# iPERDance/iPERCore

Hardware: AMD Instinct MI355X
Metric: synthesized frames/sec at 512x512 (run_imitator) (higher is better)
Workload: dtype f32; 1 GPU; run_imitator 512x512 single src/ref pair, 300-frame reference clip frame-sharded over 1 GPU(s), AttLWB-SPADE generator fp32 (BASELINE configs[1] at N = 1, configs[2] at N = 8); poses=imitate, image_size=512, frame_batch=300, frame_batch_requested=384, world_size=1, parallelism=frame-shard x1, batches_in_flight=1, weights=random-init (seeded) of the real architecture, 36,276,992 params

## Files before the change

include/lwg_hip.h:

```cpp
#ifndef LWG_HIP_H
#define LWG_HIP_H

#include <stddef.h>
#include <stdint.h>

#ifdef __cplusplus
extern "C" {
#endif

typedef void* lwg_stream_t;

#define LWG_ABI_VERSION 10
int lwg_abi_version(void);

#define LWG_MAX_TAPS 52
enum { LWG_EPI_NONE = 0, LWG_EPI_RESIDUAL = 1, LWG_EPI_SPADE = 2 };
enum { LWG_ACTIVATION_NONE = 0, LWG_ACTIVATION_RELU = 1, LWG_ACTIVATION_TANH = 2, LWG_ACTIVATION_SIGMOID = 3 };
#define LWG_ACTIVATION_RELU_MASK 5
enum { LWG_DT_F32 = 0, LWG_DT_BF16 = 1,
       LWG_DT_F32_Q4 = 2 };

typedef struct LwgConvArgs {
    const float* x0;
    const float* x1;
    int C0, C1;
    int B, H, W;
    int OH, OW;
    int M;
    int stride;
    int ntaps;
    int cshift;
    const float* w;
    int N;
    const float* bias;
    float* y;
    int YH, YW, YC, ycoff;
    int omul, ooy, oox;
    int epi;
    int act;
    const float* res;
    const float* xn;
    const float* mean;
    const float* rstd;
    int xdt;
    int ydt;
    signed char dy[LWG_MAX_TAPS];
    signed char dx[LWG_MAX_TAPS];
} LwgConvArgs;

int lwg_conv2d_nhwc_f32(const LwgConvArgs* args, lwg_stream_t stream);
size_t lwg_conv2d_ws_floats(const LwgConvArgs* args);
int lwg_conv2d_nhwc_f32_ws(const LwgConvArgs* args, float* ws, lwg_stream_t stream);
int lwg_conv_slice_count(const LwgConvArgs* args);

int lwg_conv2d_nhwc_bf16(const LwgConvArgs* args, lwg_stream_t stream);
int lwg_conv2d_winograd_f32(const LwgConvArgs* args, lwg_stream_t stream);
size_t lwg_conv2d_winograd_ws_floats(const LwgConvArgs* args);
int lwg_conv2d_winograd_f32_ws(const LwgConvArgs* args, float* ws, lwg_stream_t stream);
int lwg_conv2d_winograd_plan(const LwgConvArgs* args, int with_ws, long long* blocks, int* slices, int* nbv, int* workgroups);
int lwg_winograd_panel_f32(const float* wpanel, float* upk, int Cin, int N, const int* tap9, lwg_stream_t stream);
typedef struct LwgWinoDesc {
    const float* wpanel;
    float* upk;
    int Cin, N, first_block;
    int tap9[9];
} LwgWinoDesc;
int lwg_winograd_panels_f32(const LwgWinoDesc* descs_dev, int ndesc, int total_blocks, lwg_stream_t stream);
int lwg_conv2d_winograd4_f32(const LwgConvArgs* args, lwg_stream_t stream);
int lwg_winograd4_panel_f32(const float* wpanel, float* upk, int Cin, int N, const int* tap9, lwg_stream_t stream);
int lwg_conv2d_nhwc_bf16_hr(const LwgConvArgs* args, lwg_stream_t stream);
int lwg_conv2d_nhwc_c8_bf16(const LwgConvArgs* args, lwg_stream_t stream);
int lwg_conv_transpose4_nhwc_bf16(const LwgConvArgs* args, lwg_stream_t stream);
int lwg_conv_transpose4_nhwc_f32(const LwgConvArgs* args, lwg_stream_t stream);
int lwg_conv_transpose4_is_one_grid(const LwgConvArgs* args);
int lwg_conv_transpose4_winograd_f32(const LwgConvArgs* args, lwg_stream_t stream);

int lwg_conv2d_nhwc_f32_split(const LwgConvArgs* args, lwg_stream_t stream);

size_t lwg_conv2d_wgrad_ws_floats(int Ktot, int N, int M);
int lwg_conv2d_wgrad_nhwc_f32(const LwgConvArgs* args, const float* dy, float* dw, float* ws, lwg_stream_t stream);
int lwg_conv2d_wgrad_unpacked_f32(const LwgConvArgs* args, const float* dy, float* ws, float* dw, int D0, int D1, int KH, int KW,
                                  int transposed, const int* kidx, int cin, int nout, float* db, lwg_stream_t stream);
int lwg_colsum_nhwc_f32(const float* x, size_t rows, int C, float* out, float* ws, lwg_stream_t stream);

int lwg_act_bwd_f32(const float* dy, const float* y, size_t n, int act, float* out, lwg_stream_t stream);
int lwg_norm_fwd_nhwc_f32(const float* x, const float* mean, const float* rstd, const float* gamma, const float* beta, int gstride,
                          int B, int HW, int C, int act, float* y, lwg_stream_t stream);
int lwg_norm_bwd_nhwc_f32(const float* dy, const float* y, const float* x, const float* mean, const float* rstd,
                          const float* gamma, int gstride, int B, int HW, int C, int act, int nsplit, float* dx, float* dgamma,
                          float* dbeta, float* ws, lwg_stream_t stream);
int lwg_adam_step_f32(float* p, const float* g, float* m, float* v, size_t n, float lr, float beta1, float beta2, float eps, int t,
                      lwg_stream_t stream);
int lwg_adam_step_dev_f32(float* p, const float* g, float* m, float* v, size_t n, float lr, float beta1, float beta2, float eps,
                          int* t_dev, lwg_stream_t stream);
int lwg_pack_panel_f32(const float* w, int D0, int D1, int KH, int KW, int transposed, const int* kidx, int ntaps, int cin,
                       int cin_pad, int nout, int n_pad, float* out, lwg_stream_t stream);
int lwg_unpack_wgrad_f32(const float* dwk, int D0, int D1, int KH, int KW, int transposed, const int* kidx, int ntaps, int cin,
                         int cin_pad, int nout, int n_pad, float* dw, lwg_stream_t stream);
typedef struct LwgPackDesc {
    const float* w;
    float* out;
    int D1, KHW, transposed, ntaps, cin, cin_pad, nout, n_pad, Kp, first_block;
    int kidx[LWG_MAX_TAPS];
} LwgPackDesc;
int lwg_pack_panels_f32(const LwgPackDesc* descs_dev, int ndesc, int total_blocks, lwg_stream_t stream);
int lwg_maxpool2_fwd_nhwc_f32(const float* x, float* y, int B, int H, int W, int C, lwg_stream_t stream);
int lwg_maxpool2_bwd_nhwc_f32(const float* x, const float* dy, float* dx, int B, int H, int W, int C, lwg_stream_t stream);
int lwg_crop_resize_bilinear_f32(const float* x, const long long* box, float* y, float* valid, int N, int C, int H, int W, int OH, int OW,
                                 lwg_stream_t stream);
int lwg_crop_resize_bilinear_bwd_f32(const float* dy, const long long* box, float* dx, int N, int C, int H, int W, int OH, int OW, lwg_stream_t stream);
int lwg_prelu_f32(const float* x, const float* slope, const float* res, size_t rows, int C, float* y, lwg_stream_t stream);
int lwg_prelu_bwd_f32(const float* x, const float* slope, const float* dy, size_t rows, int C, float* dx, lwg_stream_t stream);

int lwg_instnorm_stats_nhwc_f32(const float* x, int B, int HW, int C, float eps, float* mean, float* rstd,
                                float* ws, int nsplit, lwg_stream_t stream);
int lwg_instnorm_stats_nhwc_bf16(const void* x, int B, int HW, int C, float eps, float* mean, float* rstd, float* ws, int nsplit,
                                 lwg_stream_t stream);
int lwg_instnorm_apply_nhwc_f32(const float* x, const float* mean, const float* rstd, const float* res,
                                float* y, int B, int HW, int C, int act, lwg_stream_t stream);

int lwg_flow_resize_f32(const float* T, int n, int S, int h, int w, float* out, lwg_stream_t stream);
int lwg_lwb_attention_f32(const float* q, const float* Ks, const float* Vs, const float* bk, const float* bv,
                          const float* T, float* out, int B, int ns, int h, int w, int C, int S,
                          int src_batched, lwg_stream_t stream);
int lwg_lwb_attention_bf16(const void* q, const void* Ks, const void* Vs, const float* bk, const float* bv, const float* T, void* out,
                           int B, int ns, int h, int w, int C, int S, int src_batched, lwg_stream_t stream);
int lwg_lwb_attention_x_records(int h, int w, int C, int element_size);
int lwg_lwb_attention_x_f32(const float* x, const float* Kq, const float* kappa, const float* Vs, const float* bv, const float* T,
// ... 71 lines not shown
```

ipercore_amd/_lib.py:

```python
import ctypes
import os
import re

_HERE = os.path.dirname(os.path.abspath(__file__))
LIB_PATH = os.path.join(_HERE, "liblwg_hip.so")
HEADER_PATH = os.path.join(os.path.dirname(_HERE), "include", "lwg_hip.h")

LWG_MAX_TAPS = 52
EPI_NONE, EPI_RESIDUAL, EPI_SPADE = 0, 1, 2
ACT_NONE, ACT_RELU, ACT_TANH, ACT_SIGMOID, ACT_LRELU = 0, 1, 2, 3, 4
ACT_RELU_MASK = 5
DT_F32, DT_BF16, DT_F32_Q4 = 0, 1, 2

c_f = ctypes.c_void_p
c_i = ctypes.c_int


class LwgConvArgs(ctypes.Structure):
    _fields_ = [
        ("x0", c_f), ("x1", c_f),
        ("C0", c_i), ("C1", c_i),
        ("B", c_i), ("H", c_i), ("W", c_i),
        ("OH", c_i), ("OW", c_i),
        ("M", c_i), ("stride", c_i), ("ntaps", c_i), ("cshift", c_i),
        ("w", c_f), ("N", c_i), ("bias", c_f),
        ("y", c_f), ("YH", c_i), ("YW", c_i), ("YC", c_i), ("ycoff", c_i),
        ("omul", c_i), ("ooy", c_i), ("oox", c_i),
        ("epi", c_i), ("act", c_i),
        ("res", c_f), ("xn", c_f), ("mean", c_f), ("rstd", c_f),
        ("xdt", c_i), ("ydt", c_i),
        ("dy", ctypes.c_byte * LWG_MAX_TAPS), ("dx", ctypes.c_byte * LWG_MAX_TAPS),
    ]


class LwgWinoDesc(ctypes.Structure):
    _fields_ = [("wpanel", ctypes.c_void_p), ("upk", ctypes.c_void_p), ("Cin", c_i), ("N", c_i), ("first_block", c_i), ("tap9", c_i * 9)]


class LwgPackDesc(ctypes.Structure):
    _fields_ = [("w", c_f), ("out", c_f)] + [(n, c_i) for n in ("D1", "KHW", "transposed", "ntaps", "cin", "cin_pad", "nout", "n_pad", "Kp",
                                                               "first_block")] + [("kidx", c_i * LWG_MAX_TAPS)]


_SIGS = {
    "lwg_abi_version": (c_i, []),
    "lwg_device_cu_count": (c_i, []),
    "lwg_conv2d_nhwc_f32": (c_i, [ctypes.POINTER(LwgConvArgs), c_f]),
    "lwg_conv2d_ws_floats": (ctypes.c_size_t, [ctypes.POINTER(LwgConvArgs)]),
    "lwg_conv2d_nhwc_f32_ws": (c_i, [ctypes.POINTER(LwgConvArgs), c_f, c_f]),
    "lwg_conv2d_nhwc_bf16": (c_i, [ctypes.POINTER(LwgConvArgs), c_f]),
    "lwg_conv2d_winograd_f32": (c_i, [ctypes.POINTER(LwgConvArgs), c_f]),
    "lwg_conv2d_winograd_ws_floats": (ctypes.c_size_t, [ctypes.POINTER(LwgConvArgs)]),
    "lwg_conv2d_winograd_f32_ws": (c_i, [ctypes.POINTER(LwgConvArgs), c_f, c_f]),
    "lwg_conv2d_winograd_plan": (c_i, [ctypes.POINTER(LwgConvArgs), c_i, ctypes.POINTER(ctypes.c_longlong), ctypes.POINTER(c_i), ctypes.POINTER(c_i),
                                       ctypes.POINTER(c_i)]),
    "lwg_winograd_panel_f32": (c_i, [c_f, c_f, c_i, c_i, ctypes.POINTER(c_i), c_f]),
    "lwg_winograd_panels_f32": (c_i, [c_f, c_i, c_i, c_f]),
    "lwg_conv2d_winograd4_f32": (c_i, [ctypes.POINTER(LwgConvArgs), c_f]),
    "lwg_winograd4_panel_f32": (c_i, [c_f, c_f, c_i, c_i, ctypes.POINTER(c_i), c_f]),
    "lwg_conv2d_nhwc_bf16_hr": (c_i, [ctypes.POINTER(LwgConvArgs), c_f]),
    "lwg_conv2d_nhwc_c8_bf16": (c_i, [ctypes.POINTER(LwgConvArgs), c_f]),
    "lwg_conv_transpose4_nhwc_bf16": (c_i, [ctypes.POINTER(LwgConvArgs), c_f]),
    "lwg_conv_transpose4_nhwc_f32": (c_i, [ctypes.POINTER(LwgConvArgs), c_f]),
    "lwg_conv_transpose4_winograd_f32": (c_i, [ctypes.POINTER(LwgConvArgs), c_f]),
    "lwg_conv_transpose4_is_one_grid": (c_i, [ctypes.POINTER(LwgConvArgs)]),
    "lwg_conv_slice_count": (c_i, [ctypes.POINTER(LwgConvArgs)]),
    "lwg_conv2d_nhwc_f32_split": (c_i, [ctypes.POINTER(LwgConvArgs), c_f]),
    "lwg_conv2d_wgrad_ws_floats": (ctypes.c_size_t, [c_i, c_i, c_i]),
    "lwg_conv2d_wgrad_nhwc_f32": (c_i, [ctypes.POINTER(LwgConvArgs), c_f, c_f, c_f, c_f]),
    "lwg_conv2d_wgrad_unpacked_f32": (c_i, [ctypes.POINTER(LwgConvArgs), c_f, c_f, c_f] + [c_i] * 5 + [ctypes.POINTER(ctypes.c_int), c_i, c_i, c_f, c_f]),
    "lwg_colsum_nhwc_f32": (c_i, [c_f, ctypes.c_size_t, c_i, c_f, c_f, c_f]),
    "lwg_act_bwd_f32": (c_i, [c_f, c_f, ctypes.c_size_t, c_i, c_f, c_f]),
    "lwg_norm_fwd_nhwc_f32": (c_i, [c_f, c_f, c_f, c_f, c_f, c_i, c_i, c_i, c_i, c_i, c_f, c_f]),
    "lwg_norm_bwd_nhwc_f32": (c_i, [c_f, c_f, c_f, c_f, c_f, c_f, c_i, c_i, c_i, c_i, c_i, c_i, c_f, c_f, c_f, c_f, c_f]),
    "lwg_adam_step_f32": (c_i, [c_f, c_f, c_f, c_f, ctypes.c_size_t, ctypes.c_float, ctypes.c_float, ctypes.c_float, ctypes.c_float, c_i, c_f]),
    "lwg_adam_step_dev_f32": (c_i, [c_f, c_f, c_f, c_f, ctypes.c_size_t, ctypes.c_float, ctypes.c_float, ctypes.c_float, ctypes.c_float, c_f, c_f]),
    "lwg_pack_panel_f32": (c_i, [c_f] + [c_i] * 5 + [ctypes.POINTER(ctypes.c_int)] + [c_i] * 5 + [c_f, c_f]),
    "lwg_pack_panels_f32": (c_i, [c_f, c_i, c_i, c_f]),
    "lwg_unpack_wgrad_f32": (c_i, [c_f] + [c_i] * 5 + [ctypes.POINTER(ctypes.c_int)] + [c_i] * 5 + [c_f, c_f]),
    "lwg_maxpool2_fwd_nhwc_f32": (c_i, [c_f, c_f, c_i, c_i, c_i, c_i, c_f]),
    "lwg_maxpool2_bwd_nhwc_f32": (c_i, [c_f, c_f, c_f, c_i, c_i, c_i, c_i, c_f]),
    "lwg_crop_resize_bilinear_f32": (c_i, [c_f, c_f, c_f, c_f, c_i, c_i, c_i, c_i, c_i, c_i, c_f]),
    "lwg_crop_resize_bilinear_bwd_f32": (c_i, [c_f, c_f, c_f, c_i, c_i, c_i, c_i, c_i, c_i, c_f]),
    "lwg_prelu_f32": (c_i, [c_f, c_f, c_f, ctypes.c_size_t, c_i, c_f, c_f]),
    "lwg_prelu_bwd_f32": (c_i, [c_f, c_f, c_f, ctypes.c_size_t, c_i, c_f, c_f]),
    "lwg_instnorm_stats_nhwc_f32": (c_i, [c_f, c_i, c_i, c_i, ctypes.c_float, c_f, c_f, c_f, c_i, c_f]),
    "lwg_instnorm_apply_nhwc_f32": (c_i, [c_f, c_f, c_f, c_f, c_f, c_i, c_i, c_i, c_i, c_f]),
    "lwg_lwb_attention_f32": (c_i, [c_f, c_f, c_f, c_f, c_f, c_f, c_f, c_i, c_i, c_i, c_i, c_i, c_i, c_i, c_f]),
    "lwg_lwb_attention_bf16": (c_i, [c_f, c_f, c_f, c_f, c_f, c_f, c_f, c_i, c_i, c_i, c_i, c_i, c_i, c_i, c_f]),
    "lwg_instnorm_stats_nhwc_bf16": (c_i, [c_f, c_i, c_i, c_i, ctypes.c_float, c_f, c_f, c_f, c_i, c_f]),
    "lwg_head_compose_bf16": (c_i, [c_f, c_f, c_f, ctypes.c_size_t, c_i, c_i, c_i, c_f, c_f, c_f, c_f]),
    "lwg_up4_head_compose_bf16": (c_i, [ctypes.POINTER(LwgConvArgs), c_f, c_f, ctypes.c_size_t, c_f, c_f, c_f, c_f]),
    "lwg_flow_resize_f32": (c_i, [c_f, c_i, c_i, c_i, c_i, c_f, c_f]),
    "lwg_lwb_fuse_f32": (c_i, [c_f] * 5 + [c_i] * 7 + [ctypes.c_float, ctypes.c_float, c_f]),
    "lwg_lwb_attention_x_f32": (c_i, [c_f] * 8 + [c_i] * 6 + [c_f]),
    "lwg_lwb_attention_x_bf16": (c_i, [c_f] * 8 + [c_i] * 6 + [c_f]),
    "lwg_lwb_attention_x_records": (c_i, [c_i, c_i, c_i, c_i]),
    "lwg_instnorm_finalize_ws_floats": (ctypes.c_size_t, [c_i, c_i, c_i]),
    "lwg_instnorm_finalize_f32": (c_i, [c_f, c_i, c_i, c_i, ctypes.c_float, c_f, c_f, c_f]),
    "lwg_lwb_attention_bwd_f32": (c_i, [c_f] * 10 + [c_i] * 7 + [c_f]),
    "lwg_lwb_attention_kv_f32": (c_i, [c_f] * 6 + [c_i] * 7 + [c_f]),
    "lwg_lwb_attention_kv_bwd_f32": (c_i, [c_f] * 8 + [c_i] * 7 + [c_f]),
    "lwg_rasterize_ws_bytes": (ctypes.c_size_t, [c_i, c_i, c_i]),
    "lwg_project_faces_f32": (c_i, [c_f, c_f, c_f, c_i, c_i, c_i, ctypes.c_float, c_f, c_f, c_f]),
    "lwg_rasterize_fim_wim_f32": (c_i, [c_f, c_i, c_i, c_i, ctypes.c_float, ctypes.c_float, c_f, c_f, c_f, c_f]),
    "lwg_texture_sample_f32": (c_i, [c_f, c_f, c_f, c_f, c_i, c_i, c_i, c_i, c_i, ctypes.c_float, ctypes.POINTER(ctypes.c_float), c_f, c_f]),
    "lwg_flow_compose_f32": (c_i, [c_f, c_f, c_i, c_i, c_f, c_i, c_f, c_f, c_i, c_i, c_f, c_i, c_f, c_f, c_f, c_f, c_f]),
    "lwg_bc_transform_f32": (c_i, [c_f, c_f, c_f, c_i, c_i, c_i, c_f, c_f]),
    "lwg_encode_fim_f32": (c_i, [c_f, c_f, c_i, c_i, c_i, c_i, c_f, c_f]),
    "lwg_smpl_lbs_ws_floats": (ctypes.c_size_t, [c_i, c_i, c_i]),
    "lwg_smpl_lbs_f32": (c_i, [c_f, c_i, c_f, c_i, c_i, c_f, c_i, c_f, c_f, c_i, c_f, c_f, c_f, c_f, c_f, c_f, c_i, c_i, c_i,
                               c_i, c_f, c_f, c_f, c_f, c_f]),
    "lwg_head_compose_f32": (c_i, [c_f, c_f, c_f, ctypes.c_size_t, c_i, c_i, c_i, c_f, c_f, c_f, c_f]),
    "lwg_head_compose_q4_f32": (c_i, [c_f, c_f, c_f, ctypes.c_size_t, c_i, c_i, c_i, c_f, c_f, c_f, c_f]),
    "lwg_thin_conv_f32": (c_i, [c_f, c_f, c_i, c_i, c_i, c_i, c_f, c_f]),
    "lwg_nchw_to_nhwc_f32": (c_i, [c_f, c_f, c_i, c_i, c_i, c_i, c_f]),
    "lwg_nhwc_to_nchw_f32": (c_i, [c_f, c_f, c_i, c_i, c_i, c_i, c_f]),
# ... 43 lines not shown
```

ipercore_amd/ops.py:

```python
import ctypes

import torch

from . import _lib
from ._lib import ACT_LRELU, ACT_NONE, ACT_RELU, ACT_RELU_MASK, ACT_SIGMOID, ACT_TANH, EPI_NONE, EPI_RESIDUAL, EPI_SPADE

EYE_DIST = 2.7320508075688776


def _ptr(t, dtype=torch.float32):
    if t is None:
        return None
    if not t.is_cuda:
        raise RuntimeError("ipercore_amd ops need CUDA (HIP) tensors: the MI355X path has no CPU fallback")
    if t.dtype != dtype:
        raise TypeError(f"expected {dtype}, got {t.dtype}")
    if not t.is_contiguous():
        raise ValueError("tensor must be contiguous")
    return t.data_ptr()


CONV_PRECISION = "fp32"


class conv_precision(object):

    def __init__(self, mode):
        assert mode in ("fp32", "bf16", "split", "winograd", "winograd2x2")
        self.mode = mode

    def __enter__(self):
        global CONV_PRECISION, WINO4
        self.prev = CONV_PRECISION, WINO4
        if self.mode == "winograd2x2":
            CONV_PRECISION, WINO4 = "winograd", False
        else:
            CONV_PRECISION = self.mode

    def __exit__(self, *exc):
        global CONV_PRECISION, WINO4
        CONV_PRECISION, WINO4 = self.prev


CONV_HOOK = None


def _stream():
    return torch.cuda.current_stream().cuda_stream


class ConvSpec:
    __slots__ = ("w", "bias", "N", "Cin", "ntaps", "dy", "dx", "stride", "cshift", "omul", "ooy", "oox", "algo_kn", "_w16v2", "_w16hr", "_w16x3", "_w16c8", "_w16up", "_w32up", "_wwino", "_wwino_t", "_wwino4")

    def __init__(self, w, bias, N, Cin, taps, stride=1, omul=1, ooy=0, oox=0, algo_kn=None):
        self.w, self.bias, self.N, self.Cin = w, bias, int(N), int(Cin)
        self.algo_kn = int(algo_kn) if algo_kn is not None else len(taps) * int(Cin) * int(N)
        self.ntaps = len(taps)
        self.dy = [int(t[0]) for t in taps]
        self.dx = [int(t[1]) for t in taps]
        self.stride, self.omul, self.ooy, self.oox = stride, omul, ooy, oox
        self._w16v2 = None
        self._w16hr = None
        self._w16x3 = None
        self._w16c8 = None
        self._w16up = None
        self._w32up = None
        self._wwino = None
        self._wwino_t = None
        self._wwino4 = None
        self.cshift = 0
        if self.Cin % 32 != 0:
            q = self.Cin // 4
            assert q in (1, 2, 4), "small-Cin path handles Cin in {4, 8, 16}"
            self.cshift = q.bit_length() - 1


def _w16v2(spec):
    if spec._w16v2 is None or spec._w16v2.device != spec.w.device:
        K4, N, _ = spec.w.shape
        cin, nt = spec.Cin, spec.ntaps
        assert cin % 64 == 0 and K4 * 4 == nt * cin, (cin, nt, K4)
        wk = spec.w.permute(0, 2, 1).reshape(cin // 64, 2, nt, 32, N)
        wk = wk.permute(0, 2, 1, 3, 4).reshape(cin // 64 * nt, 64, N)
        rows = wk.permute(0, 2, 1).reshape(cin // 64 * nt, N, 8, 8)
        n = torch.arange(N, device=spec.w.device)
        slot = torch.arange(8, device=spec.w.device)
        src = slot[None, :] ^ ((n[:, None] >> 1) & 7)
        rows = torch.gather(rows, 2, src[None, :, :, None].expand(rows.shape[0], N, 8, 8))
        spec._w16v2 = rows.reshape(cin // 64 * nt, N, 64).contiguous().to(torch.bfloat16)
    return spec._w16v2


def _hr_eligible(spec, x0, y, out_hw):
    if not BF16_HR or spec.stride != 1 or spec.ntaps not in (9, 4) or spec.N % 64 != 0 or spec.Cin % 64 != 0:
        return False
    if any(abs(d) > 1 for d in spec.dy) or any(abs(d) > 1 for d in spec.dx):
        return False
    OH, OW = ((y.shape[1], y.shape[2]) if spec.omul == 1 else (y.shape[1] // spec.omul, y.shape[2] // spec.omul)) if out_hw is None else out_hw
    return (OH, OW) == (x0.shape[1], x0.shape[2])


def _hr_tap_order(spec):
    return sorted(range(spec.ntaps), key=lambda t: (spec.dy[t], spec.dx[t]))


def _w16hr(spec, spade):
    key = bool(spade)
    if spec._w16hr is None or spec._w16hr[0] != key or spec._w16hr[1].device != spec.w.device:
        K4, N, _ = spec.w.shape
        cin, nt = spec.Cin, spec.ntaps
        wk = spec.w.permute(0, 2, 1).reshape(cin // 64, 2, nt, 32, N).permute(0, 2, 1, 3, 4).reshape(cin // 64, nt, 64, N)
        wk = wk[:, _hr_tap_order(spec)].reshape(cin // 64 * nt, 64, N)
        bias = spec.bias
        if spade:
            j = torch.arange(N, device=spec.w.device)
            q, r = j // 32, j % 32
            ch = 16 * q + (r % 16)
            old = 64 * (ch // 32) + (ch % 32) + 32 * (r // 16)
            wk = wk[:, :, old]
            bias = None if bias is None else bias[old].contiguous()
        panel = wk.reshape(cin // 64 * nt, 4, 16, N).permute(0, 1, 3, 2).contiguous().to(torch.bfloat16)
# ... 202 lines not shown
        kind = "split"
        _lib.check(_lib.lib().lwg_conv2d_nhwc_f32_split(a, _stream()), "lwg_conv2d_nhwc_f32_split")
    else:
        nws = _lib.lib().lwg_conv2d_ws_floats(a) if splitk else 0
        if nws:
            ws = torch.empty(nws, device=x0.device, dtype=torch.float32)
            _lib.check(_lib.lib().lwg_conv2d_nhwc_f32_ws(a, _ptr(ws), _stream()), "lwg_conv2d_nhwc_f32_ws")
        else:
            _lib.check(_lib.lib().lwg_conv2d_nhwc_f32(a, _stream()), "lwg_conv2d_nhwc_f32")
    if CONV_HOOK is not None:
        _hook_end(a, spec, epi, kind, sliced, extra)
    return y


WINO_UP4 = True
F32_UP4 = True
BF16_UP4 = True


def _parity_specs_ok(specs):
    s0 = specs[0]
    return (len(specs) == 4 and all(s.ntaps == 4 and s.omul == 2 and s.stride == 1 and (s.ooy, s.oox) == (i >> 1, i & 1) and s.N == s0.N and s.Cin == s0.Cin
                                    and [(dy - (i >> 1), dx - (i & 1)) for dy, dx in zip(s.dy, s.dx)] == list(zip(s0.dy, s0.dx)) for i, s in enumerate(specs)))


def _wwino_t(specs):
    s0 = specs[0]
    U = s0._wwino_t
    if U is not None and U.device == s0.w.device:
        return U
    Cin, N = s0.Cin, s0.N
    G = torch.tensor([[1.0, 0.0], [1.0, 1.0], [0.0, 1.0]], dtype=torch.float64, device=s0.w.device)
    parts = []
    for par, sp in enumerate(specs):
        py, px = par >> 1, par & 1
        W = sp.w.double().permute(0, 2, 1).reshape(4 * Cin, N)
        W = W.view(Cin // 32, 4, 32, N).permute(1, 0, 2, 3).reshape(4, Cin, N)
        g = torch.zeros(2, 2, Cin, N, dtype=torch.float64, device=W.device)
        for t, (dy, dx) in enumerate(zip(sp.dy, sp.dx)):
            g[dy - (py - 1), dx - (px - 1)] = W[t]
        u = torch.einsum("ar,rqcn,bq->abcn", G, g, G)
        if py:
            u[0] = -u[0]
        if px:
            u[:, 0] = -u[:, 0]
        parts.append(u.reshape(9, Cin, N))
    U9 = torch.stack(parts).float()
    U = torch.cat([U9[:, 0:4].permute(0, 2, 3, 1).reshape(4, Cin, 4 * N), U9[:, 4:8].permute(0, 2, 3, 1).reshape(4, Cin, 4 * N), U9[:, 8]], dim=2)
    U = U.view(4, Cin // 8, 4, 2, 9 * N).contiguous()
    s0._wwino_t = U
    return U


class _FusedTransposeSpec(object):

    def __init__(self, s0, panel):
        self.N, self.Cin, self.ntaps, self.stride, self.omul = 4 * s0.N, s0.Cin, 16, 1, 2
        self.algo_kn, self.w = 4 * s0.algo_kn, panel


def conv_transpose2d(x, specs, y, act=ACT_NONE, splitk=False, out_hw=None, q4=False):
    s0 = specs[0]
    if (BF16_UP4 and BF16_HR and x.dtype == torch.bfloat16 and y.dtype == torch.bfloat16 and len(specs) == 4 and s0.Cin in (64, 128)
            and s0.N % 64 == 0 and all(s.ntaps == 4 and s.omul == 2 and (s.ooy, s.oox) == (i >> 1, i & 1) for i, s in enumerate(specs))):
        a = conv_args(x, s0, y, act=act)
        panel = getattr(s0, "_w16up", None)
        if panel is None or panel.device != s0.w.device:
            panel = torch.stack([_w16hr(s, False)[0] for s in specs]).contiguous()
            s0._w16up = panel
        a.w = _ptr(panel, torch.bfloat16)
        if CONV_HOOK is not None:
            whole = _FusedTransposeSpec(s0, panel)
            CONV_HOOK(True, a.M, whole, EPI_NONE, None)
        _lib.check(_lib.lib().lwg_conv_transpose4_nhwc_bf16(a, _stream()), "lwg_conv_transpose4_nhwc_bf16")
        if CONV_HOOK is not None:
            _hook_end(a, whole, EPI_NONE, "up4")
        return y
    if (WINO_UP4 and CONV_PRECISION == "winograd" and not splitk and out_hw is None and x.is_cuda and x.dtype == torch.float32 and y.dtype == torch.float32
            and s0.Cin % 32 == 0 and s0.N % 32 == 0 and _parity_specs_ok(specs)):
        a = conv_args(x, s0, y, act=act, q4=q4)
        panel = _wwino_t(specs)
        a.w = _ptr(panel)
        if CONV_HOOK is not None:
            whole = _FusedTransposeSpec(s0, panel)
            CONV_HOOK(True, a.M, whole, EPI_NONE, None)
        _lib.check(_lib.lib().lwg_conv_transpose4_winograd_f32(a, _stream()), "lwg_conv_transpose4_winograd_f32")
        if CONV_HOOK is not None:
            _hook_end(a, whole, EPI_NONE, "winograd_up4", False)
        return y
    if (F32_UP4 and x.is_cuda and x.dtype == torch.float32 and y.dtype == torch.float32 and CONV_PRECISION in ("fp32", "winograd") and s0.Cin % 32 == 0
            and _parity_specs_ok(specs)):
        a = conv_args(x, s0, y, act=act, q4=q4)
        if _lib.lib().lwg_conv_transpose4_is_one_grid(a):
            panel = getattr(s0, "_w32up", None)
            if panel is None or panel.device != s0.w.device:
                panel = torch.stack([s.w.reshape(-1) for s in specs]).contiguous()
                s0._w32up = panel
            a.w = _ptr(panel)
            if CONV_HOOK is not None:
                whole = _FusedTransposeSpec(s0, panel)
                CONV_HOOK(True, a.M, whole, EPI_NONE, None)
            _lib.check(_lib.lib().lwg_conv_transpose4_nhwc_f32(a, _stream()), "lwg_conv_transpose4_nhwc_f32")
            if CONV_HOOK is not None:
                _hook_end(a, whole, EPI_NONE, "up4")
            return y
    for s in specs:
        conv2d(x, s, y, act=act, splitk=splitk, out_hw=None if out_hw is None else out_hw(s), q4=q4)
    return y


def instnorm_stats(x, mean, rstd, ws, eps=1e-5, nsplit=None):
    B, H, W, C = x.shape
    HW = H * W
    if nsplit is None:
        nsplit = max(1, min(64, HW // 64))
    assert ws.numel() >= B * C * nsplit * 3
    if x.dtype == torch.bfloat16:
        _lib.check(_lib.lib().lwg_instnorm_stats_nhwc_bf16(_ptr(x, torch.bfloat16), B, HW, C, eps, _ptr(mean), _ptr(rstd), _ptr(ws), nsplit,
                                                            _stream()), "lwg_instnorm_stats_nhwc_bf16")
        return
    _lib.check(_lib.lib().lwg_instnorm_stats_nhwc_f32(_ptr(x), B, HW, C, eps, _ptr(mean), _ptr(rstd), _ptr(ws), nsplit,
                                                       _stream()), "lwg_instnorm_stats_nhwc_f32")


def instnorm_apply(x, mean, rstd, y, act=ACT_NONE, res=None):
    B, H, W, C = x.shape
    _lib.check(_lib.lib().lwg_instnorm_apply_nhwc_f32(_ptr(x), _ptr(mean), _ptr(rstd), _ptr(res), _ptr(y), B, H * W, C, act,
                                                       _stream()), "lwg_instnorm_apply_nhwc_f32")
    return y


def flow_resize(T, h, w):
    B, ns, S = T.shape[0], T.shape[1], T.shape[2]
    T = T.contiguous()
    out = torch.empty(B, ns, h, w, 2, device=T.device, dtype=torch.float32)
    _lib.check(_lib.lib().lwg_flow_resize_f32(_ptr(T), B * ns, S, h, w, _ptr(out), _stream()), "lwg_flow_resize_f32")
    return out


# ... 659 lines not shown
```

Baseline: 1188 frames/s.

## Add F(2x2)/F(2x4) Winograd kernel for fused transposed-conv upsampling on large maps

Adds a new HIP kernel that computes the four-parity transposed convolution with a mixed Winograd transform, 3 points in y and 5 in x (15 forms instead of 9). Each tile then yields more output per multiply, cutting MFMA work per output pixel. It also adds a matching weight-panel transform in Python, and routes inputs with spatial area of at least 64x64 to the new kernel. The cost is more LDS traffic, register pressure and a larger weight panel, plus some fp32 rounding from the non-trivial transform constants.

```diff
diff --git a/include/lwg_hip.h b/include/lwg_hip.h
--- a/include/lwg_hip.h
+++ b/include/lwg_hip.h
@@ -74,6 +74,8 @@
 int lwg_conv_transpose4_nhwc_f32(const LwgConvArgs* args, lwg_stream_t stream);
 int lwg_conv_transpose4_is_one_grid(const LwgConvArgs* args);
 int lwg_conv_transpose4_winograd_f32(const LwgConvArgs* args, lwg_stream_t stream);
+
+int lwg_conv_transpose4_winograd24_f32(const LwgConvArgs* args, lwg_stream_t stream);
 
 int lwg_conv2d_nhwc_f32_split(const LwgConvArgs* args, lwg_stream_t stream);
 
diff --git a/ipercore_amd/_lib.py b/ipercore_amd/_lib.py
--- a/ipercore_amd/_lib.py
+++ b/ipercore_amd/_lib.py
@@ -63,6 +63,7 @@
     "lwg_conv_transpose4_nhwc_bf16": (c_i, [ctypes.POINTER(LwgConvArgs), c_f]),
     "lwg_conv_transpose4_nhwc_f32": (c_i, [ctypes.POINTER(LwgConvArgs), c_f]),
     "lwg_conv_transpose4_winograd_f32": (c_i, [ctypes.POINTER(LwgConvArgs), c_f]),
+    "lwg_conv_transpose4_winograd24_f32": (c_i, [ctypes.POINTER(LwgConvArgs), c_f]),
     "lwg_conv_transpose4_is_one_grid": (c_i, [ctypes.POINTER(LwgConvArgs)]),
     "lwg_conv_slice_count": (c_i, [ctypes.POINTER(LwgConvArgs)]),
     "lwg_conv2d_nhwc_f32_split": (c_i, [ctypes.POINTER(LwgConvArgs), c_f]),
diff --git a/ipercore_amd/csrc/convt_winograd24.hip b/ipercore_amd/csrc/convt_winograd24.hip
--- /dev/null
+++ b/ipercore_amd/csrc/convt_winograd24.hip
@@ -0,0 +1,451 @@
+#include <hip/hip_runtime.h>
+#include "lwg_common.h"
+#include "lwg_conv_args.h"
+
+#define WG_THREADS 512
+#define TPBY 8
+#define TPBX 4
+#define NPATCH 32
+#define NBT 32
+#define KS 8
+#define HALO 18
+#define PLANE (HALO * HALO)
+#define RAW_FLOATS (KS * PLANE)
+#define VSTR NPATCH
+#define NFORM 45
+#define VS_FLOATS (NFORM * KS * VSTR)
+#define DUMP_OFF (2 * RAW_FLOATS + 2 * VS_FLOATS)
+#define DUMP_FLOATS (WG_THREADS + 3 * PLANE + RAW_FLOATS)
+#define LOOP_FLOATS (DUMP_OFF + DUMP_FLOATS)
+#define OROW 36
+#define OUT_FLOATS (32 * 32 * OROW)
+#define BIAS_OFF (LOOP_FLOATS > OUT_FLOATS ? LOOP_FLOATS : OUT_FLOATS)
+#define WINO_OOB 0xC0000000u
+#define WSB() __builtin_amdgcn_sched_barrier(0)
+#ifndef CTW24_TSWAP
+#define CTW24_TSWAP 1
+#endif
+#ifndef CTW24_TSPREAD
+#define CTW24_TSPREAD 0
+#endif
+
+#ifdef LWG_CTW24_TS
+#define CTS24(i, v) do { if (lab_bi == 1 && lane == 0) reinterpret_cast<unsigned long long*>(const_cast<float*>(a.res))[((size_t)blockIdx.x * 8 + wid) * 8 + (i)] = (v); } while (0)
+#else
+#define CTS24(i, v) do { } while (0)
+#endif
+
+namespace {
+
+template <int V> struct IntT { static constexpr int value = V; };
+
+__device__ __forceinline__ int ctw24_slot(int ly, int lx) {
+    return ((lx & 7) * 4 + (lx >> 3)) ^ (((ly >> 2) & 1) << 2);
+}
+
+__device__ __forceinline__ floatx4 ctw24_buf_load(__amdgpu_buffer_rsrc_t r, unsigned voff, unsigned soff) {
+    return __builtin_bit_cast(floatx4, __builtin_amdgcn_raw_buffer_load_b128(r, (int)voff, (int)soff, 0));
+}
+
+__device__ __forceinline__ void ctw24_cols(const float (&c)[6], float (&v)[9]) {
+    const float d12 = c[2] - c[1], d23 = c[3] - c[2], d34 = c[4] - c[3];
+    const float e13 = c[3] - c[1], e24 = c[4] - c[2];
+    v[0] = (c[0] - c[2]) + 2.f * e13;
+    v[1] = d12 + 2.f * c[3];
+    v[2] = 2.f * d23 - d12;
+    v[3] = e13;
+    v[4] = 2.f * e24 - e13;
+    v[5] = d23 + 2.f * c[4];
+    v[6] = 2.f * d34 - d23;
+    v[7] = e24;
+    v[8] = 2.f * (c[5] - c[3]) - e24;
+}
+
+}
+
+__global__ __launch_bounds__(WG_THREADS, 1) void lwg_convt_winograd24_kernel(const LwgConvArgs a) {
+    extern __shared__ __attribute__((aligned(16))) float smem[];
+    const int wid = __builtin_amdgcn_readfirstlane(threadIdx.x >> 6);
+    const int H = a.H, W = a.W, Cin = a.C0, N = a.N;
+    float* const raw0 = smem;
+    const int tid = threadIdx.x, lane = tid & 63;
+    const int bx = (W + 2 * TPBY - 1) / (2 * TPBY), by = (H + 2 * TPBY - 1) / (2 * TPBY);
+    const int tiles = bx * by * a.B;
+    const int total = tiles * (N / NBT);
+    int blk = blockIdx.x;
+    const int nst = Cin / KS;
+    const __amdgpu_buffer_rsrc_t ru = __builtin_amdgcn_make_buffer_rsrc(const_cast<float*>(a.w), 0, (int)(240u * (unsigned)Cin * (unsigned)N), 0x00020000);
+    const int par = wid & 3, py = par >> 1, px = par & 1;
+    const int hh = wid >> 2;
+    floatx16 acc[9];
+    int b, x0, y0, n0;
+    __amdgpu_buffer_rsrc_t rx0;
+    unsigned voff0[2];
+    unsigned uvoff, uvoffc;
+    const int ncb = N / NBT;
+    const bool xcd = (gridDim.x & 7u) == 0 && (ncb == 2 || ncb == 4 || ncb == 8) && (int)gridDim.x < total && tiles >= (int)gridDim.x / ncb;
+    const int xg = (int)gridDim.x / ncb;
+    const int xr = (int)(((blockIdx.x & 7u) / (unsigned)ncb) * (gridDim.x >> 3) + (blockIdx.x >> 3));
+    auto has_block = [&](int id) -> bool {
+        return xcd ? (id / (int)gridDim.x) * xg + xr < tiles : id < total;
+    };
+    auto setup = [&](int id) {
+        int cb, t;
+        if (xcd) {
+            cb = (int)(blockIdx.x & 7u) & (ncb - 1);
+            t = __builtin_amdgcn_readfirstlane((id / (int)gridDim.x) * xg + xr);
+        } else {
+            cb = __builtin_amdgcn_readfirstlane(id / tiles);
+            t = __builtin_amdgcn_readfirstlane(id - cb * tiles);
+        }
+        b = __builtin_amdgcn_readfirstlane(t / (bx * by));
+        t -= b * bx * by;
+        x0 = (t % bx) * 2 * TPBY;
+        y0 = (t / bx) * 2 * TPBY;
+        n0 = cb * NBT;
+        rx0 = __builtin_amdgcn_make_buffer_rsrc(const_cast<float*>(a.x0 + (size_t)b * H * W * Cin), 0, (int)((unsigned)(H * W) * (unsigned)Cin * 4u), 0x00020000);
+#pragma unroll
+        for (int q = 0; q < 2; ++q) {
+            const int i = tid + WG_THREADS * q;
+            const int pix = i >> 1, half = i & 1, hy = pix / HALO, hx = pix - hy * HALO;
+            const int gy = y0 - 1 + hy, gx = x0 - 1 + hx;
+            const bool in = i < PLANE * 2 && gy >= 0 && gy < H && gx >= 0 && gx < W;
+            voff0[q] = in ? (unsigned)((gy * W + gx) * Cin + 4 * half) * 4u : WINO_OOB;
+        }
+        const unsigned kh = (unsigned)(lane >> 5) * 15u * (unsigned)N, n = (unsigned)(n0 + (lane & 31));
+        uvoff = (kh + (hh ? 9u * N : 0u) + 4u * n) * 4u;
+        uvoffc = (kh + (hh ? 13u : 8u) * N + n) * 4u;
+    };
+    setup(blk);
+    int wst[2];
+#pragma unroll
+    for (int q = 0; q < 2; ++q) {
+        const int i = tid + WG_THREADS * q;
+        wst[q] = i < PLANE * 2 ? 4 * (i & 1) * PLANE + (i >> 1) : DUMP_OFF + tid;
+    }
+    floatx4 rreg[2];
+    auto rld1 = [&](int st, int q) -> floatx4 { return ctw24_buf_load(rx0, voff0[q], (unsigned)(st * KS) * 4u); };
+    auto rst1 = [&](int buf, int q, floatx4 v) {
+        float* dst = raw0 + buf * RAW_FLOATS + wst[q];
+#pragma unroll
+        for (int k = 0; k < 4; ++k) dst[k * PLANE] = v[k];
+    };
+    floatx4 ufr[4][3];
+    const unsigned ukk = (unsigned)N * 120u;
+    const unsigned upar = (unsigned)par * (unsigned)nst * 4u * ukk;
+    const unsigned ubo = (unsigned)N * 16u;
+    auto uld1 = [&](int st, int kk, int j, int h) -> floatx4 {
+        const unsigned so = upar + (unsigned)(st * 4 + kk) * ukk;
+        floatx4 r;
+        if (h == 0) {
+            if (j < 2) return ctw24_buf_load(ru, uvoff, so + (j ? ubo : 0u));
+            r[0] = __builtin_bit_cast(float, __builtin_amdgcn_raw_buffer_load_b32(ru, (int)uvoffc, (int)so, 0));
+            r[1] = r[2] = r[3] = 0.f;
+            return r;
+        }
+        if (j == 0) return ctw24_buf_load(ru, uvoff, so);
+        r[0] = r[1] = r[2] = r[3] = 0.f;
+        if (j == 1) {
+            r[0] = __builtin_bit_cast(float, __builtin_amdgcn_raw_buffer_load_b32(ru, (int)uvoffc, (int)so, 0));
+            r[1] = __builtin_bit_cast(float, __builtin_amdgcn_raw_buffer_load_b32(ru, (int)uvoffc, (int)(so + 4u * (unsigned)N), 0));
+        }
+        return r;
+    };
+    const int patch = tid & 31, tc = (tid >> 5) & 7;
+    const int pty = patch >> 2, ptx = patch & 3;
+    unsigned dbs[2];
+    unsigned vbs[2];
+    unsigned fbs[2];
+#pragma unroll
+    for (int u = 0; u < 2; ++u) {
+        dbs[u] = (unsigned)(u * RAW_FLOATS + tc * PLANE + (2 * pty + ((hh ^ CTW24_TSWAP) ? 0 : 2)) * HALO + 4 * ptx) >> 1;
+        asm volatile("" : "+v"(dbs[u]));
+        dbs[u] <<= 1;
+        vbs[u] = (unsigned)(2 * RAW_FLOATS + u * VS_FLOATS + ((hh ^ CTW24_TSWAP) ? 0 : 27) * KS * VSTR + tc * VSTR + patch);
+        asm volatile("" : "+v"(vbs[u]));
+        fbs[u] = (unsigned)(2 * RAW_FLOATS + u * VS_FLOATS + (18 * py + 4 * px + 3 * hh) * KS * VSTR + (lane >> 5) * VSTR + (lane & 31));
+        asm volatile("" : "+v"(fbs[u]));
+    }
+    float fb[2][9];
+
+    auto kloop = [&](auto HC) {
+        constexpr int HV = decltype(HC)::value;
+        constexpr int NP = HV ? 6 : 9;
+        constexpr int NU = HV ? 2 : 3;
+        constexpr int TV = HV ^ CTW24_TSWAP;
+        constexpr int NR = TV ? 3 : 2;
+        auto fragread = [&](int buf, int kk) {
+#pragma unroll
+            for (int q = 0; q < NP; ++q) fb[kk & 1][q] = smem[fbs[buf] + ((9 * (q / NU) + q % NU) * KS + 2 * kk) * VSTR];
+        };
+        auto rowforms = [&](const float (&dd)[3][6], float (&t)[3][6]) {
+#pragma unroll
+            for (int j = 0; j < 6; ++j) {
+                if (TV) {
+                    t[0][j] = dd[0][j] - dd[1][j];
+                    t[1][j] = dd[1][j];
+                    t[2][j] = dd[2][j] - dd[1][j];
+                } else {
+                    t[0][j] = dd[0][j];
+                    t[1][j] = dd[1][j] - dd[0][j];
+                }
+            }
+        };
+        auto tstore = [&](int buf, int i, const float (&t)[3][6]) {
+            float v[9];
+            ctw24_cols(t[i], v);
+            float* dst = smem + vbs[buf] + (9 * i) * KS * VSTR;
+#pragma unroll
+            for (int f = 0; f < 9; ++f) dst[f * KS * VSTR] = v[f];
+        };
+        auto ddread = [&](int buf, int i, float (&dd)[3][6]) {
+#pragma unroll
+            for (int j = 0; j < 6; ++j) dd[i][j] = smem[dbs[buf] + i * HALO + j];
+        };
+        auto iteration = [&](int s, auto SET, auto NXT) {
+            constexpr int set = decltype(SET)::value;
+            constexpr bool nxt = decltype(NXT)::value != 0;
+            const int s3 = s + 3 < nst ? s + 3 : nst - 1;
+            float dd[3][6], t[3][6];
+            auto mf = [&](int kk, int q) {
+                acc[q] = __builtin_amdgcn_mfma_f32_32x32x2f32(ufr[kk][q >> 2][q & 3], fb[kk & 1][q], acc[q], 0, 0, 0);
+                WSB();
+            };
+            auto uldn = [&](int kk) {
+                constexpr int NJ = HV ? 2 : 3;
+                if (kk < 2) {
+#pragma unroll
+                    for (int j = 0; j < NJ; ++j) ufr[kk + 2][j] = uld1(s, kk + 2, j, HV);
+                } else if (nxt) {
+#pragma unroll
+                    for (int j = 0; j < NJ; ++j) ufr[kk - 2][j] = uld1(s + 1, kk - 2, j, HV);
+                }
+                WSB();
+            };
+            uldn(0);
+            fragread(set, 1);
+            WSB();
+            mf(0, 0);
+            if (nxt) { rst1(set, 0, rreg[0]); rreg[0] = rld1(s3, 0); }
+            WSB();
+            mf(0, 1);
+            if (nxt) { rst1(set, 1, rreg[1]); rreg[1] = rld1(s3, 1); }
+            WSB();
+#pragma unroll
+            for (int q = 2; q < NP; ++q) {
+                mf(0, q);
+                if (nxt && q - 2 < NR) ddread(set ^ 1, q - 2, dd);
+                WSB();
+            }
+            if (nxt) rowforms(dd, t);
+            WSB();
+            uldn(1);
+            fragread(set, 2);
+            WSB();
+#pragma unroll
+            for (int q = 0; q < NP; ++q) {
+                mf(1, q);
+                if (nxt && !CTW24_TSPREAD && q < NR) tstore(set ^ 1, q, t);
+                if (nxt && CTW24_TSPREAD && q % 2 == 0 && q / 2 < (NR + 1) / 2) tstore(set ^ 1, q / 2, t);
+                WSB();
+            }
+            uldn(2);
+            fragread(set, 3);
+            WSB();
+#pragma unroll
+            for (int q = 0; q < NP; ++q) {
+                mf(2, q);
+                if (nxt && CTW24_TSPREAD && q % 2 == 0 && (NR + 1) / 2 + q / 2 < NR) tstore(set ^ 1, (NR + 1) / 2 + q / 2, t);
+                WSB();
+            }
+            uldn(3);
+#pragma unroll
+            for (int q = 0; q < NP / 2; ++q) mf(3, q);
+            __syncthreads();
+            if (nxt) fragread(set ^ 1, 0);
+            WSB();
+#pragma unroll
+            for (int q = NP / 2; q < NP; ++q) mf(3, q);
+        };
+        {
+            float dd[3][6], t[3][6];
+#pragma unroll
+            for (int i = 0; i < NR; ++i) ddread(0, i, dd);
+            rowforms(dd, t);
+#pragma unroll
+            for (int i = 0; i < NR; ++i) tstore(0, i, t);
+        }
+        __syncthreads();
+        fragread(0, 0);
+#pragma unroll
+        for (int q = 0; q < NP; ++q)
+#pragma unroll
+            for (int r = 0; r < 16; ++r) acc[q][r] = 0.f;
+        int s = 0;
+        for (; s + 2 < nst; s += 2) {
+            iteration(s, IntT<0>(), IntT<1>());
+            iteration(s + 1, IntT<1>(), IntT<1>());
+        }
+        iteration(s, IntT<0>(), IntT<0 + 1>());
+        iteration(s + 1, IntT<1>(), IntT<0>());
+    };
+
+    floatx4 r0[2], r1[2];
+    float bq;
+    auto issue_loads = [&]() {
+        bq = a.bias ? a.bias[n0 + (tid & 31)] : 0.f;
+#pragma unroll
+        for (int q = 0; q < 2; ++q) {
+            r0[q] = rld1(0, q);
+            r1[q] = rld1(1, q);
+        }
+#pragma unroll
+        for (int j = 0; j < 3; ++j) {
+            ufr[0][j] = uld1(0, 0, j, hh);
+            ufr[1][j] = uld1(0, 1, j, hh);
+        }
+#pragma unroll
+        for (int q = 0; q < 2; ++q) rreg[q] = rld1(nst > 2 ? 2 : 1, q);
+    };
+    issue_loads();
+#ifdef LWG_CTW24_TS
+    int lab_bi = 0;
+#endif
+    for (;;) {
+#pragma unroll
+    for (int q = 0; q < 2; ++q) {
+        rst1(0, q, r0[q]);
+        rst1(1, q, r1[q]);
+    }
+    if (tid < 32) smem[BIAS_OFF + tid] = bq;
+    __syncthreads();
+    CTS24(0, (unsigned long long)__builtin_amdgcn_s_getreg(63492));
+    CTS24(1, __builtin_readcyclecounter());
+    if (hh == 0) kloop(IntT<0>()); else kloop(IntT<1>());
+    CTS24(2, __builtin_readcyclecounter());
+    const int eb = b, ex0 = x0, ey0 = y0, en0 = n0;
+    int tide = tid;
+    asm volatile("" : "+v"(tide));
+    const int lanee = tide & 63;
+    const int ety = (lanee & 31) >> 2, etx = lanee & 3;
+    const int chl = 4 * (lanee >> 5);
+    auto opix = [&](int ia, int ib) -> float* {
+        const int ly = 4 * ety + 2 * ia + py, lx = 8 * etx + 2 * ib + px;
+        return smem + (ly * 32 + ctw24_slot(ly, lx)) * OROW + chl;
+    };
+    __syncthreads();
+    if (hh == 1) {
+#pragma unroll
+        for (int g = 0; g < 4; ++g)
+#pragma unroll
+            for (int ia = 0; ia < 2; ++ia) {
+                floatx4 o[4];
+#pragma unroll
+                for (int k = 0; k < 4; ++k) {
+                    const int r = 4 * g + k;
+                    const float s3 = acc[2 * ia][r] + acc[2 * ia + 2][r], s4 = acc[2 * ia + 1][r] + acc[2 * ia + 3][r];
+                    o[0][k] = s3;
+                    o[1][k] = 0.5f * s3;
+                    o[2][k] = 0.25f * s3;
+                    o[3][k] = __builtin_fmaf(0.125f, s3, s4);
+                }
+#pragma unroll
+                for (int ib = 0; ib < 4; ++ib) *reinterpret_cast<floatx4*>(opix(ia, ib) + 8 * g) = o[ib];
+            }
+    }
+    __syncthreads();
+    CTS24(3, __builtin_readcyclecounter());
+    if (hh == 0) {
+        lwg_act_dispatch(a.act, [&](auto ACTC) {
+        constexpr int EA = decltype(ACTC)::value;
+#pragma unroll
+        for (int g = 0; g < 4; ++g) {
+            const floatx4 bv = *reinterpret_cast<const floatx4*>(smem + BIAS_OFF + 8 * g + chl);
+#pragma unroll
+            for (int ia = 0; ia < 2; ++ia) {
+                floatx4 o[4];
+#pragma unroll
+                for (int k = 0; k < 4; ++k) {
+                    const int r = 4 * g + k;
+                    const float s0 = acc[3 * ia][r] + acc[3 * ia + 3][r], s1 = acc[3 * ia + 1][r] + acc[3 * ia + 4][r];
+                    const float s2 = acc[3 * ia + 2][r] + acc[3 * ia + 5][r];
+                    o[0][k] = (s0 + s1) + s2;
+                    o[1][k] = s1 - s2;
+                    o[2][k] = s1 + s2;
+                    o[3][k] = s1 - s2;
+                }
+#pragma unroll
+                for (int ib = 0; ib < 4; ++ib) {
+                    floatx4* dst = reinterpret_cast<floatx4*>(opix(ia, ib) + 8 * g);
+                    const floatx4 pv = *dst;
+                    floatx4 y;
+#pragma unroll
+                    for (int k = 0; k < 4; ++k) y[k] = lwg_act_c<EA>((o[ib][k] + pv[k]) + bv[k], a.act);
+                    *dst = y;
+                }
+            }
+        }
+        });
+    }
+    const int nblk = blk + (int)gridDim.x;
+    const bool more = has_block(nblk);
+    setup(more ? nblk : blk);
+    issue_loads();
+    __syncthreads();
+    const int oy0 = 2 * ey0, ox0 = 2 * ex0;
+    const size_t plane = (size_t)a.YH * a.YW;
+    typedef unsigned int ctw_u4 __attribute__((ext_vector_type(4)));
+    if (a.ydt == LWG_DT_F32_Q4) {
+        const int lx = tide & 31, cq = (tide >> 5) & 7, lyh = tide >> 8;
+        const __amdgpu_buffer_rsrc_t ry = __builtin_amdgcn_make_buffer_rsrc(a.y + (size_t)eb * (size_t)(a.YC >> 2) * plane * 4, 0,
+                                                                            (int)((unsigned)(a.YC >> 2) * (unsigned)plane * 16u), 0x00020000);
+        const unsigned yv = ox0 + lx < a.YW ? (unsigned)(((((a.ycoff + en0) >> 2) + cq) * (int)plane + (oy0 + lyh) * a.YW + ox0 + lx) * 16) : WINO_OOB;
+        const unsigned rowpair = (unsigned)a.YW * 32u;
+#pragma unroll
+        for (int pass = 0; pass < 16; ++pass) {
+            const int ly = lyh + 2 * pass;
+            const ctw_u4 v = *reinterpret_cast<const ctw_u4*>(smem + (ly * 32 + ctw24_slot(ly, lx)) * OROW + 4 * cq);
+            __builtin_amdgcn_raw_buffer_store_b128(v, ry, (int)(oy0 + 2 * pass < a.YH ? yv + (unsigned)pass * rowpair : WINO_OOB), 0, 0);
+        }
+    } else {
+        const int cq = tide & 7, lx = (tide >> 3) & 31, lyh = tide >> 8;
+        const __amdgpu_buffer_rsrc_t ry = __builtin_amdgcn_make_buffer_rsrc(a.y + (size_t)eb * plane * a.YC, 0, (int)((unsigned)plane * (unsigned)a.YC * 4u), 0x00020000);
+        const unsigned yv = ox0 + lx < a.YW ? (unsigned)((((oy0 + lyh) * a.YW + ox0 + lx) * a.YC + a.ycoff + en0 + 4 * cq) * 4) : WINO_OOB;
+        const unsigned rowpair = (unsigned)a.YW * (unsigned)a.YC * 8u;
+#pragma unroll
+        for (int pass = 0; pass < 16; ++pass) {
+            const int ly = lyh + 2 * pass;
+            const ctw_u4 v = *reinterpret_cast<const ctw_u4*>(smem + (ly * 32 + ctw24_slot(ly, lx)) * OROW + 4 * cq);
+            __builtin_amdgcn_raw_buffer_store_b128(v, ry, (int)(yv + (unsigned)pass * rowpair), 0, 0);
+        }
+    }
+    CTS24(4, __builtin_readcyclecounter());
+    if (!more) break;
+#ifdef LWG_CTW24_TS
+    ++lab_bi;
+#endif
+    blk = nblk;
+    __syncthreads();
+    }
+}
+
+extern "C" int lwg_conv_transpose4_winograd24_f32(const LwgConvArgs* pa, lwg_stream_t stream_) {
+    hipStream_t stream = reinterpret_cast<hipStream_t>(stream_);
+    if (!pa) return (int)hipErrorInvalidValue;
+    const LwgConvArgs& a = *pa;
+    if (!a.x0 || !a.w || !a.y || a.M <= 0 || a.ntaps != 4 || a.stride != 1 || a.omul != 2 || a.C0 <= 0 || (a.C0 % (2 * KS)) != 0 || a.C1 != 0 ||
+        a.N <= 0 || (a.N % NBT) != 0 || a.OH != a.H || a.OW != a.W || a.YH != 2 * a.H || a.YW != 2 * a.W || a.xdt != LWG_DT_F32 ||
+        (a.ydt != LWG_DT_F32 && a.ydt != LWG_DT_F32_Q4) || a.M != a.B * a.H * a.W || a.epi != LWG_EPI_NONE || a.act == LWG_ACT_RELU_MASK ||
+        a.ycoff < 0 || (a.ycoff % 4) != 0 || (a.YC % 4) != 0 || a.ycoff + a.N > a.YC)
+        return (int)hipErrorInvalidValue;
+    if ((unsigned long long)a.H * a.W * a.C0 * 4ull >= (unsigned long long)WINO_OOB || 240ull * a.C0 * a.N >= 0x7fffffffull) return (int)hipErrorInvalidValue;
+    if ((unsigned long long)a.YH * a.YW * a.YC * 4ull + 32ull * a.YW * a.YC * 4ull >= (unsigned long long)WINO_OOB) return (int)hipErrorInvalidValue;
+    const size_t lds = (size_t)(BIAS_OFF + 32) * 4;
+    static unsigned long long done = 0;
+    if (hipError_t e = lwg_allow_dynamic_lds(reinterpret_cast<const void*>(lwg_convt_winograd24_kernel), lds, done); e != hipSuccess) return (int)e;
+    const int bx = (a.W + 2 * TPBY - 1) / (2 * TPBY), by = (a.H + 2 * TPBY - 1) / (2 * TPBY);
+    const long total = (long)bx * by * a.B * (a.N / NBT);
+    const int cus = lwg_device_cus();
+    hipLaunchKernelGGL(lwg_convt_winograd24_kernel, dim3((unsigned)(LWG_WINO_PERSIST && total > cus ? cus : total)), dim3(WG_THREADS), lds, stream, a);
+    return (int)hipGetLastError();
+}
diff --git a/ipercore_amd/ops.py b/ipercore_amd/ops.py
--- a/ipercore_amd/ops.py
+++ b/ipercore_amd/ops.py
@@ -50,7 +50,7 @@
 
 
 class ConvSpec:
-    __slots__ = ("w", "bias", "N", "Cin", "ntaps", "dy", "dx", "stride", "cshift", "omul", "ooy", "oox", "algo_kn", "_w16v2", "_w16hr", "_w16x3", "_w16c8", "_w16up", "_w32up", "_wwino", "_wwino_t", "_wwino4")
+    __slots__ = ("w", "bias", "N", "Cin", "ntaps", "dy", "dx", "stride", "cshift", "omul", "ooy", "oox", "algo_kn", "_w16v2", "_w16hr", "_w16x3", "_w16c8", "_w16up", "_w32up", "_wwino", "_wwino_t", "_wwino_t24", "_wwino4")
 
     def __init__(self, w, bias, N, Cin, taps, stride=1, omul=1, ooy=0, oox=0, algo_kn=None):
         self.w, self.bias, self.N, self.Cin = w, bias, int(N), int(Cin)
@@ -67,6 +67,7 @@
         self._w32up = None
         self._wwino = None
         self._wwino_t = None
+        self._wwino_t24 = None
         self._wwino4 = None
         self.cshift = 0
         if self.Cin % 32 != 0:
@@ -375,6 +376,45 @@
     return U
 
 
+_G_X24 = ((1.0, 0.0), (0.5, 0.5), (-1.0 / 6.0, 1.0 / 6.0), (-8.0 / 3.0, -4.0 / 3.0), (0.0, 0.5))
+
+
+def _wwino_t24(specs):
+    s0 = specs[0]
+    U = s0._wwino_t24
+    if U is not None and U.device == s0.w.device:
+        return U
+    Cin, N = s0.Cin, s0.N
+    Gy = torch.tensor([[1.0, 0.0], [1.0, 1.0], [0.0, 1.0]], dtype=torch.float64, device=s0.w.device)
+    Gx = torch.tensor(_G_X24, dtype=torch.float64, device=s0.w.device)
+    parts = []
+    for par, sp in enumerate(specs):
+        py, px = par >> 1, par & 1
+        W = sp.w.double().permute(0, 2, 1).reshape(4 * Cin, N)
+        W = W.view(Cin // 32, 4, 32, N).permute(1, 0, 2, 3).reshape(4, Cin, N)
+        g = torch.zeros(2, 2, Cin, N, dtype=torch.float64, device=W.device)
+        for t, (dy, dx) in enumerate(zip(sp.dy, sp.dx)):
+            g[dy - (py - 1), dx - (px - 1)] = W[t]
+        u = torch.einsum("ar,rqcn,bq->abcn", Gy, g, Gx)
+        if py:
+            u[0] = -u[0]
+        parts.append(torch.cat([u[:, :3].reshape(9, Cin, N), u[:, 3:].reshape(6, Cin, N)]))
+    U15 = torch.stack(parts).float()
+    quad = lambda lo, hi: U15[:, lo:hi].permute(0, 2, 3, 1).reshape(4, Cin, (hi - lo) * N)
+    U = torch.cat([quad(0, 4), quad(4, 8), U15[:, 8], quad(9, 13), U15[:, 13], U15[:, 14]], dim=2)
+    U = U.view(4, Cin // 8, 4, 2, 15 * N).contiguous()
+    s0._wwino_t24 = U
+    return U
+
+
+WINO_UP4_24 = True
+WINO_UP4_24_MIN_HW = 64 * 64
+
+
+def _up4_24(x):
+    return WINO_UP4_24 and x.shape[1] * x.shape[2] >= WINO_UP4_24_MIN_HW
+
+
 class _FusedTransposeSpec(object):
 
     def __init__(self, s0, panel):
@@ -402,12 +442,16 @@
     if (WINO_UP4 and CONV_PRECISION == "winograd" and not splitk and out_hw is None and x.is_cuda and x.dtype == torch.float32 and y.dtype == torch.float32
             and s0.Cin % 32 == 0 and s0.N % 32 == 0 and _parity_specs_ok(specs)):
         a = conv_args(x, s0, y, act=act, q4=q4)
-        panel = _wwino_t(specs)
+        f24 = _up4_24(x)
+        panel = _wwino_t24(specs) if f24 else _wwino_t(specs)
         a.w = _ptr(panel)
         if CONV_HOOK is not None:
             whole = _FusedTransposeSpec(s0, panel)
             CONV_HOOK(True, a.M, whole, EPI_NONE, None)
-        _lib.check(_lib.lib().lwg_conv_transpose4_winograd_f32(a, _stream()), "lwg_conv_transpose4_winograd_f32")
+        if f24:
+            _lib.check(_lib.lib().lwg_conv_transpose4_winograd24_f32(a, _stream()), "lwg_conv_transpose4_winograd24_f32")
+        else:
+            _lib.check(_lib.lib().lwg_conv_transpose4_winograd_f32(a, _stream()), "lwg_conv_transpose4_winograd_f32")
         if CONV_HOOK is not None:
             _hook_end(a, whole, EPI_NONE, "winograd_up4", False)
         return y
```

After: 1212 frames/s, median of 6. 2.1% higher.
